# bxh1/VIDO-SLAM

Hardware: AMD Instinct MI355X
Metric: frames/sec end-to-end (flow+depth+track+local-BA) at 640x480; BA iters/sec (higher is better)
Workload: dtype f32

## Files before the change

### include/vido_c.h

```cpp
#ifndef VIDO_C_H
#define VIDO_C_H
#include <stdint.h>
#include <stddef.h>
#ifdef __cplusplus
extern "C" {
#endif

#define VIDO_OK              0
#define VIDO_E_INVALID      -1
#define VIDO_E_NO_DEVICE    -2
#define VIDO_E_HIP          -3
#define VIDO_E_CAPACITY     -4
#define VIDO_E_NOMEM        -5

#define VIDO_MAX_LEVELS 16

typedef struct vido_ctx vido_ctx;

typedef struct vido_keypoint { float x, y, size, angle, response; int32_t octave; } vido_keypoint;

typedef struct vido_config {
    int32_t device;
    int32_t width, height;
    int32_t max_batch;
// ... 126 lines not shown
    double* H_T;
    double* dyn_xyz;
    const int32_t* dyn_cam; const double* dyn_meas;
    const int32_t* tern_prev; const int32_t* tern_cur; const int32_t* tern_H;
    const int32_t* sm_i; const int32_t* sm_j;
    double info_dyn, info_tern, info_smooth, huber_dyn, huber_tern, huber_smooth;
} vido_ba_dynamic;
int vido_ba_optimize_dynamic(vido_ctx* ctx, vido_ba_problem* prob, vido_ba_dynamic* dyn, vido_ba_result* result,
                             vido_allreduce_fn allreduce, void* user);

int vido_correlation(vido_ctx* ctx, const float* first, const float* second, int B, int C, int H, int W, int stride,
                     float* out, int on_device);
int vido_det_order(vido_ctx* ctx, const float* scores, const long long* labels, const int* n_det, float confidence, int cap, long long* order, long long* labels_out, long long* n_live);
int vido_roi_levels(vido_ctx* ctx, const float* boxes, int n, float k_min, float k_max, int* out);
int vido_mask_logit_select(vido_ctx* ctx, const float* feat, const float* w, const float* b, const long long* labels, float* out, int n, int c, int hw, int classes);
int vido_bias_act(vido_ctx* ctx, float* x, const float* bias, int N, int C, int H, int W, float slope);
int vido_bias_unary(vido_ctx* ctx, float* x, const float* bias, int N, int C, int H, int W, int kind);
int vido_upcat_reflect(vido_ctx* ctx, const float* x, const float* skip, int C1, int C2, int h, int w, float* out);
int vido_minmax_norm_u16(vido_ctx* ctx, const float* d, const float* mm, int64_t n, int32_t* out);
int vido_bias_res_act(vido_ctx* ctx, float* x, const float* bias, const float* res, int N, int C, int H, int W, float slope);
int vido_area_feed(vido_ctx* ctx, const uint8_t* bgr, int H, int W, float* out, int OH, int OW, float div);
int vido_backwarp(vido_ctx* ctx, const float* x, const float* flow, int B, int C, int H, int W, float* out);
int vido_deconv4s2_depthwise(vido_ctx* ctx, const float* x, const float* weight, int B, int C, int H, int W, float input_slope, float* out);

int vido_conv1x1_supported(int cin, int cout, int hw);
int vido_conv1x1_layout(int cin, int cout, int hw);
int vido_conv1x1_set_arith(int arith);
int vido_conv1x1_range_flag(vido_ctx* ctx, int reset);
int vido_conv1x1_bias_act(vido_ctx* ctx, const float* x, const float* w_packed, const float* bias, const float* residual, float* y, int cin, int cout, int hw, float slope);
int vido_deconv2x2_supported(int n, int cin, int cout, int h, int w);
int vido_deconv2x2_bias_act(vido_ctx* ctx, const float* x, const float* w_packed, const float* bias, float* y, int n, int cin, int cout, int h, int w, float slope);
int vido_conv1x1_bias_up2_act(vido_ctx* ctx, const float* x, const float* w_packed, const float* bias, const float* residual_half, float* y, int cin, int cout, int h, int w, float slope);

int vido_conv_kxk_c2(vido_ctx* ctx, const float* x, const float* w, const float* bias, const float* residual, float* y, int cin, int k, int h, int w_);
int vido_conv1x1_skinny(vido_ctx* ctx, const float* x, const float* w_packed, const float* bias, const float* residual, float* y, int cin, int cout, long long hw, float slope);

int vido_conv_direct_supported(int cin, int cout, int h, int w, int kh, int kw, int sh, int sw, int ph, int pw);
long long vido_conv_direct_packed_floats(int cin, int cout, int kh, int kw);
int vido_conv_direct_pack(const float* w, int cin, int cout, int kh, int kw, float* w_packed);
int vido_conv_direct_bias_act(vido_ctx* ctx, const float* x, const float* w_packed, const float* bias, float* y, int n, int cin, int cout, int h, int w,
                              int kh, int kw, int sh, int sw, int ph, int pw, float slope);

int vido_wino3x3_supported(int cin, int cout, int h, int w);
int vido_wino3x3_fills_chip(int n, int cout, int h, int w, int min_wgs);
long long vido_wino3x3_packed_floats(int cin, int cout);
int vido_wino3x3_pack(const float* w, int cin, int cout, float* u_packed);
int vido_wino3x3_bias_act(vido_ctx* ctx, const float* x, const float* u_packed, const float* bias, float* y, int n, int cin, int cout, int h, int w, float slope);
int vido_wino3x3_form(int n, int cin, int cout, int h, int w);
int vido_fc_h_splitk(int rows, int k, int outs);
int vido_fc_h(vido_ctx* ctx, const float* x, const void* w_packed, const float* bias, float* part, float* y, int rows, int k, int outs, float slope);
int vido_conv3x3_h_supported(int n, int cin, int cout, int h, int w);
int vido_conv3x3_h_workgroups(int n, int cout, int h, int w);
int vido_conv3x3_h_bias_act(vido_ctx* ctx, const float* x, const void* w_packed, const float* bias, float* y, int n, int cin, int cout, int h, int w, float slope);
long long vido_wino3x3_packed_floats_form(int cin, int cout, int form);
int vido_wino3x3_pack_form(const float* w, int cin, int cout, int form, float* u_packed);
int vido_wino3x3_bias_act_form(vido_ctx* ctx, const float* x, const float* u_packed, const float* bias, float* y, int n, int cin, int cout, int h, int w, float slope, int form);
int vido_gconv3x3_supported(int H, int W, int cpg_in, int cpg_out);
int64_t vido_gconv3x3_packed_size(int groups, int cpg_in, int cpg_out);
int vido_gconv3x3_bias_act(vido_ctx* ctx, const float* x, const float* in_bias, const float* w_packed, const float* bias, float* y, int groups, int cpg_in, int cpg_out, int H, int W, float slope);
int vido_gconv3x3_s2_supported(int H, int W, int cpg_in, int cpg_out);
int vido_gconv3x3_s2_bias_act(vido_ctx* ctx, const float* x, const float* w_packed, const float* bias, float* y, int groups, int cpg_in, int cpg_out, int H, int W, float slope);
int vido_lfn_reg_front(vido_ctx* ctx, const float* im1, const float* im2, const float* flow, const float* mean, float scale, int B, int C, int H, int W, float* out, int out_channels);
int vido_lfn_reg_tail(vido_ctx* ctx, const float* dist, const float* flow, const float* wx, const float* bx, const float* wy, const float* by, int B, int K, int H, int W, float* out);
int vido_roi_align(vido_ctx* ctx, const float* feat, int B, int C, int H, int W, const float* rois, int n_rois,
                   float spatial_scale, int pooled_h, int pooled_w, int sampling_ratio, float* out, int on_device);
int vido_nms(vido_ctx* ctx, const float* boxes_xyxy, const float* scores, int n, float thresh, int32_t* keep_out,
             int32_t* n_keep, int on_device);
int vido_nms_grouped(vido_ctx* ctx, const float* boxes_xyxy, const float* scores, const int32_t* groups, int n, float thresh,
                     int32_t* keep_out, int32_t* n_keep, int on_device);
int vido_nms_segments(vido_ctx* ctx, const float* boxes_xyxy, const int32_t* groups, const int32_t* seg_off, const int32_t* seg_n, int n_seg, int max_n, int total,
                      float thresh, int32_t* keep_out, int32_t* n_keep);
int vido_roi_align_fpn(vido_ctx* ctx, const float* const feat[4], const int H[4], const int W[4], const float scale[4], int C, const float* boxes, const int32_t* level,
                       int n, int pooled_h, int pooled_w, int sampling_ratio, float* out);
int vido_nchw_to_nhwc(vido_ctx* ctx, const float* src, int B, int C, int H, int W, float* dst);
int vido_roi_align_fpn_nhwc(vido_ctx* ctx, const float* const feat[4], const int H[4], const int W[4], const float scale[4], int C, const float* boxes, const int32_t* level,
                            int n, int pooled_h, int pooled_w, int sampling_ratio, float* out);
int vido_bawin_create(vido_ctx* ctx, int cap_frames, int cap_features);
int vido_bawin_push_frame(vido_ctx* ctx, int frame, int n, const double* meas, const float* xyz, const int32_t* asso);
int vido_bawin_set_labels(vido_ctx* ctx, int n, const int32_t* quads);
int vido_bawin_solve(vido_ctx* ctx, int start, int N, vido_ba_problem* prob, vido_ba_result* res, int32_t* n_obs_out, int32_t* n_pt_out);
int vido_bawin_read_points(vido_ctx* ctx, int frame, int n, float* xyz_out);
int vido_rpn_select(vido_ctx* ctx, int n_levels, const float* const* logits, const float* const* deltas, const int* h, const int* w, const int* stride, const float* cell_anchors,
                    int A, int K, int img_w, int img_h, float* boxes_out, float* scores_out, int32_t* n_out);
int vido_rpn_merge(vido_ctx* ctx, const float* boxes, const float* scores, const int32_t* keep, const int32_t* cnt, int n_levels, int K, int post_nms_top_n, int n_final,
                   float* out_boxes, float* out_scores, int32_t* n_valid);
int vido_det_class_sort(vido_ctx* ctx, const float* prob, const float* deltas, const float* proposals, const float* objectness, int N, int nc, float thresh, const float weights[4],
                        int img_w, int img_h, float* seg_boxes, int32_t* order, int32_t* seg_n);
int vido_det_select(vido_ctx* ctx, const float* prob, const float* seg_boxes, const int32_t* order, const int32_t* keep, const int32_t* cnt, int N, int nc, int detections_per_img, int cap,
                    int32_t* scratch, float* out_boxes, float* out_scores, int64_t* out_labels, int32_t* n_det);
int vido_mask_label_image(vido_ctx* ctx, const float* masks, const float* boxes, const int64_t* labels, int n, int M, int padding, float thresh, int H, int W, uint8_t* out);
int vido_box_decode(vido_ctx* ctx, const float* deltas, const float* boxes, int n, int k, const float weights[4],
                    float* out, int on_device);

int vido_pnp_ransac(vido_ctx* ctx, const float* pts3d, const float* pts2d, int n, double fx, double fy, double cx, double cy,
                    int max_iters, double reproj_err, double confidence, uint64_t seed, double T_out[16], uint8_t* inlier_mask,
                    int32_t* n_inliers);

int vido_pnp_ransac_batch(vido_ctx* ctx, int n_prob, const float* const* pts3d, const float* const* pts2d, const int32_t* n, double fx, double fy, double cx, double cy,
                          int max_iters, double reproj_err, double confidence, const uint64_t* seeds, double* T_out, uint8_t* const* inlier_mask, int32_t* n_inliers);

typedef struct vido_host_maps { const int32_t* mask; const float* depth; const float* flow; int32_t width, height; } vido_host_maps;
float vido_depth_noise(float z, unsigned seed);
int vido_undistort_points(const float* xy, int n, const float K[4], const float dist[5], float* xy_out);
int vido_renew_static(const vido_host_maps* maps, const float* stat_xy, int n_stat, const int32_t* TM_sta, int n_tm, const float* sample_xy, int n_sample,
                      int max_num, int32_t* src_out, int32_t* inlier_out, float* flow_out, int cap, int32_t* n_out);
int vido_renew_objects(const vido_host_maps* maps, const float* obj_xy, const int32_t* obj_label, int n_obj_pts,
// ... 48 lines not shown
```

### vido-slam_amd/csrc/conv3x3h.hip

```cpp
#include "common.hpp"
#include <type_traits>

namespace {
typedef float f32x16 __attribute__((ext_vector_type(16)));
typedef float f32x2 __attribute__((ext_vector_type(2)));
typedef _Float16 f16x8 __attribute__((ext_vector_type(8)));
typedef _Float16 f16x2 __attribute__((ext_vector_type(2)));
typedef unsigned u32x4 __attribute__((ext_vector_type(4)));

#define C3_OOB 0x40000000u
#define C3_WSLOT 24576
#define C3_RBW 3
#define C3_WPIX(BR) (((BR) + 2) * 18)
#define C3_XP(BR) ((16 * C3_WPIX(BR) + 511) / 512)
#define C3_RAW(BR) (C3_XP(BR) * 8 * 256)
#define C3_PLANE(BR) (C3_WPIX(BR) * 32)
#define C3_PBUF(BR) (2 * C3_PLANE(BR))
#define C3_LDS(BR) (C3_RBW * C3_WSLOT + C3_RAW(BR) + 2 * C3_PBUF(BR))

struct C3Args { const float* x; const void* wp; const float* bias; float* y; int N, Cin, Cout, H, W, nby, nbx, mt, total, nchunk; float slope; unsigned wbytes; unsigned* range_flag; };

template <int RPW, int CG>
__global__ __launch_bounds__(512) void k_conv3x3_h(C3Args A)
{
    constexpr int BR = 16 / CG, MT = 32 * RPW * CG, WPIX = C3_WPIX(BR), XP = C3_XP(BR), RAWB = C3_RAW(BR), PLANE = C3_PLANE(BR), PBUF = C3_PBUF(BR), CK = (WPIX * 8 + 511) / 512, NMM = 9 * RPW, NRD = 2 * RPW + 2;
    extern __shared__ __attribute__((aligned(16))) char c3_lds[];
    char* L = c3_lds;
    const int tid = threadIdx.x, lane = tid & 63, w = __builtin_amdgcn_readfirstlane(tid >> 6);
    const int per = gridDim.x >> 3, item = (blockIdx.x & 7) * per + (blockIdx.x >> 3);
    if (item >= A.total) return;
    const int nt = item / A.mt, mtile = item - nt * A.mt, m0 = mtile * MT;
    const int bpi = A.nby * A.nbx, n = nt / bpi, brem = nt - n * bpi, by = brem / A.nbx, bx = brem - by * A.nbx, Y0 = by * BR, X0 = bx * 16;
    const int rp = CG == 1 ? w : (w & 3), rb0 = CG == 1 ? 0 : RPW * (w >> 2);
    const int hw = A.H * A.W, nsteps = A.nchunk * 3;

    const __amdgpu_buffer_rsrc_t wr = __builtin_amdgcn_make_buffer_rsrc((void*)A.wp, 0, A.wbytes, 0x00020000);
    const unsigned avo = 16u * (unsigned)lane;
    unsigned abase[3], avq[3];
#pragma unroll
    for (int q = 0; q < 3; q++) { const int i = w + 8 * q, rb = i / 6, rem = i - 6 * rb; abase[q] = 1024u * (unsigned)(((m0 >> 5) + rb) * A.nchunk * 18 + rem); avq[q] = rb < RPW * CG ? avo : 0x80000000u; }
    unsigned xvo[11];
#pragma unroll
    for (int j = 0; j < XP; j++) {
        const int e = 64 * (8 * j + w) + lane, ch = e / WPIX, rem = e - ch * WPIX, row = rem / 18, col = rem - row * 18, gy = Y0 - 1 + row, gx = X0 - 1 + col;
        xvo[j] = (e < 16 * WPIX && gy >= 0 && gy < A.H && gx >= 0 && gx < A.W) ? 4u * (unsigned)(ch * hw + gy * A.W + gx) : C3_OOB;
    }
    const unsigned ximg = 4u * (unsigned)n * (unsigned)A.Cin * (unsigned)hw, ximg_end = ximg + 4u * (unsigned)A.Cin * (unsigned)hw, xchunk = 64u * (unsigned)hw;
    char* const RAW = L + C3_RBW * C3_WSLOT;
    char* const PL = RAW + RAWB;
    auto issue_w = [&](int s, int slot) {
        char* S = L + slot * C3_WSLOT + w * 1024;
        const unsigned so = 6144u * (unsigned)s;
#pragma unroll
        for (int q = 0; q < 3; q++) __builtin_amdgcn_raw_ptr_buffer_load_lds(wr, (__attribute__((address_space(3))) void*)(S + q * 8192), 16, avq[q], abase[q] + so, 0, 0);
    };
    auto issue_x = [&](int c) {
        const unsigned so = ximg + xchunk * (unsigned)c;
        const __amdgpu_buffer_rsrc_t xc = __builtin_amdgcn_make_buffer_rsrc((void*)((const char*)A.x + so), 0, ximg_end - so, 0x00020000);
#pragma unroll
        for (int j = 0; j < XP; j++) __builtin_amdgcn_raw_ptr_buffer_load_lds(xc, (__attribute__((address_space(3))) void*)(RAW + (8 * j + w) * 256), 4, xvo[j], 0, 0, 0);
    };
    float xmax = 0.f;
    const f32x2 k2048 = {2048.f, 2048.f};
    auto convert = [&](int buf) {
        const float* R = (const float*)RAW;
        unsigned* P = (unsigned*)(PL + buf * PBUF);
#pragma unroll
        for (int k = 0; k < CK; k++) {
            const int idx = tid + 512 * k;
            if (k < CK - 1 || idx < WPIX * 8) {
                const int q = idx / WPIX, pix = idx - q * WPIX;
                const f32x2 v = {R[(2 * q) * WPIX + pix], R[(2 * q + 1) * WPIX + pix]};
                const f16x2 h = __builtin_convertvector(v, f16x2);
                f32x2 vs, r;
                asm("v_pk_mul_f32 %0, %1, %2" : "=v"(vs) : "v"(v), "v"(k2048));
                asm("v_fma_mix_f32 %0, %1, %2, %3 op_sel_hi:[1,0,0]" : "=v"(r.x) : "v"(h), "s"(-2048.f), "v"(vs.x));
                asm("v_fma_mix_f32 %0, %1, %2, %3 op_sel:[1,0,0] op_sel_hi:[1,0,0]" : "=v"(r.y) : "v"(h), "s"(-2048.f), "v"(vs.y));
                const f16x2 l = __builtin_convertvector(r, f16x2);
                P[pix * 8 + q] = __builtin_bit_cast(unsigned, h); P[PLANE / 4 + pix * 8 + q] = __builtin_bit_cast(unsigned, l);
                xmax = __builtin_elementwise_maximum(__builtin_elementwise_maximum(xmax, __builtin_fabsf(v.x)), __builtin_fabsf(v.y));
            }
        }
    };

    f32x16 acc[RPW], acl[RPW];
#pragma unroll
    for (int rb = 0; rb < RPW; rb++)
#pragma unroll
        for (int r = 0; r < 16; r++) { acc[rb][r] = 0.f; acl[rb][r] = 0.f; }
    typedef const __attribute__((address_space(3))) char* lds_c;
    const unsigned a_lane = 16u * (unsigned)lane;
    const unsigned b_lane = (unsigned)(C3_RBW * C3_WSLOT + RAWB) + 32u * (unsigned)((2 * rp + ((lane & 31) >> 4)) * 18 + (lane & 15)) + 16u * (unsigned)(lane >> 5);

    issue_x(0); issue_w(0, 0); issue_w(min(1, nsteps - 1), 1);
    asm volatile("s_waitcnt vmcnt(6) lgkmcnt(0)\n\ts_barrier" ::: "memory");
    convert(0);
    int slot = 0;
    u32x4 a[2][RPW][2], b[2][2];
    auto step = [&](auto dy_c, auto nbuf_c, int pbuf, auto&& copies) {
        constexpr int dy = decltype(dy_c)::value, NBUF = decltype(nbuf_c)::value;
        lds_c Ab = (lds_c)(L + slot * C3_WSLOT) + a_lane;
        lds_c Bb = (lds_c)L + b_lane + pbuf * PBUF + dy * (18 * 32);
        auto ld = [&](int dx, int set) {
#pragma unroll
            for (int rb = 0; rb < RPW; rb++)
#pragma unroll
                for (int pl = 0; pl < 2; pl++) a[set][rb][pl] = *(const __attribute__((address_space(3))) u32x4*)(Ab + (((rb0 + rb) * 3 + dx) * 2 + pl) * 1024);
#pragma unroll
            for (int pl = 0; pl < 2; pl++) b[set][pl] = *(const __attribute__((address_space(3))) u32x4*)(Bb + dx * 32 + pl * PLANE);
        };
        __builtin_amdgcn_sched_barrier(0);
        ld(0, 0);
        copies();
#pragma unroll
        for (int dx = 0; dx < 3; dx++) {
            if (dx < 2) ld(dx + 1, (dx + 1) & 1);
#pragma unroll
            for (int term = 0; term < 3; term++) {
                constexpr int PA[3] = {0, 1, 0}, PB[3] = {1, 0, 0};
#pragma unroll
                for (int rb = 0; rb < RPW; rb++) {
                    f32x16& d = term == 2 ? acc[rb] : acl[rb];
                    d = __builtin_amdgcn_mfma_f32_32x32x16_f16(__builtin_bit_cast(f16x8, a[dx & 1][rb][PA[term]]), __builtin_bit_cast(f16x8, b[dx & 1][PB[term]]), d, 0, 0, 0);
                }
            }
        }
        __builtin_amdgcn_sched_group_barrier(0x100, NRD, 0);
#pragma unroll
        for (int i = 0; i < NMM; i++) {
            __builtin_amdgcn_sched_group_barrier(0x008, 1, 0);
            if (i < 2 * NRD) __builtin_amdgcn_sched_group_barrier(0x100, 1, 0);
            if (i >= 1 && i < 1 + NBUF) __builtin_amdgcn_sched_group_barrier(0x020, 1, 0);
        }
        __builtin_amdgcn_sched_barrier(0);
    };
    for (int c = 0; c < A.nchunk; c++) {
        const int pbuf = c & 1, cn = min(c + 1, A.nchunk - 1);
        asm volatile("s_waitcnt vmcnt(3) lgkmcnt(0)\n\ts_barrier" ::: "memory");
        step(std::integral_constant<int, 0>{}, std::integral_constant<int, 3 + XP>{}, pbuf, [&] { const int sf = slot == 0 ? C3_RBW - 1 : slot - 1; issue_w(min(3 * c + 2, nsteps - 1), sf); issue_x(cn); });
        slot = slot + 1 == C3_RBW ? 0 : slot + 1;
        asm volatile("s_waitcnt vmcnt(%0) lgkmcnt(0)\n\ts_barrier" :: "n"(3 + XP) : "memory");
        step(std::integral_constant<int, 1>{}, std::integral_constant<int, 3>{}, pbuf, [&] { const int sf = slot == 0 ? C3_RBW - 1 : slot - 1; issue_w(min(3 * c + 3, nsteps - 1), sf); });
        slot = slot + 1 == C3_RBW ? 0 : slot + 1;
        asm volatile("s_waitcnt vmcnt(3) lgkmcnt(0)\n\ts_barrier" ::: "memory");
        step(std::integral_constant<int, 2>{}, std::integral_constant<int, 3>{}, pbuf, [&] { const int sf = slot == 0 ? C3_RBW - 1 : slot - 1; issue_w(min(3 * c + 4, nsteps - 1), sf); });
        convert(pbuf ^ 1);
        slot = slot + 1 == C3_RBW ? 0 : slot + 1;
    }
    asm volatile("s_waitcnt vmcnt(0) lgkmcnt(0)" ::: "memory");
#pragma unroll
    for (int rb = 0; rb < RPW; rb++) acc[rb] += acl[rb] * 0x1p-11f;
    if (!(xmax < 65504.f) && A.range_flag) atomicOr(A.range_flag, 1u);

    const float* wsc = (const float*)((const char*)A.wp + (size_t)A.nchunk * 16 * 18 * A.Cout * 2);
    const int p = lane & 31, Y = Y0 + 2 * rp + (p >> 4), X = X0 + (p & 15);
    const bool inside = Y < A.H && X < A.W;
    float* yb = A.y + (size_t)n * A.Cout * hw + (size_t)Y * A.W + X;
#pragma unroll
    for (int rb = 0; rb < RPW; rb++) {
        float bv[16], sv[16];
#pragma unroll
        for (int r = 0; r < 16; r++) { const int co = m0 + 32 * (rb0 + rb) + 8 * (r >> 2) + 4 * (lane >> 5) + (r & 3); bv[r] = A.bias ? A.bias[co] : 0.f; sv[r] = wsc[co]; }
        if (inside) {
#pragma unroll
            for (int r = 0; r < 16; r++) {
                const int co = m0 + 32 * (rb0 + rb) + 8 * (r >> 2) + 4 * (lane >> 5) + (r & 3);
                const float v = acc[rb][r] * sv[r] + bv[r];
                yb[(size_t)co * hw] = fmaxf(v, v * A.slope);
            }
        }
    }
}
}

extern "C" {

int vido_conv3x3_h_supported(int n, int cin, int cout, int h, int w)
{
    const long long cp = (cin + 15) / 16 * 16;
    return n >= 1 && cin >= 1 && (cout == 32 || cout == 64 || (cout >= 128 && cout % 128 == 0)) && h >= 1 && w >= 1 && 4ll * n * cin * h * w < (1ll << 30) && 4ll * n * cout * h * w < (1ll << 30)
           && 36ll * cp * cout < (1ll << 31);
}

#define C3_MIN16 190
static int c3_block_rows(int n, int cout, int h, int w)
{
    static const int force = [] { const char* e = getenv("VIDO_CONV3X3_H_ROWS"); return e ? atoi(e) : 0; }();
    if (cout == 32) return 16;
    if (force == 16 || force == 8) return force;
    const int mt = cout >= 128 ? cout / 128 : 1;
    return n * ((h + 15) / 16) * ((w + 15) / 16) * mt >= C3_MIN16 ? 16 : 8;
}
int vido_conv3x3_h_workgroups(int n, int cout, int h, int w) { const int br = c3_block_rows(n, cout, h, w); return n * ((h + br - 1) / br) * ((w + 15) / 16) * (cout >= 128 ? cout / 128 : 1); }

int vido_conv3x3_h_bias_act(vido_ctx* ctx, const float* x, const void* w_packed, const float* bias, float* y, int n, int cin, int cout, int h, int w, float slope)
{
    if (!ctx) return VIDO_E_INVALID;
    if (!x || !w_packed || !y || x == y || !vido_conv3x3_h_supported(n, cin, cout, h, w) || slope < 0.f || slope > 1.f || (((uintptr_t)x | (uintptr_t)y) & 3) || ((uintptr_t)w_packed & 15))
        return vido_set_error(ctx, VIDO_E_INVALID, "conv3x3_h: no kernel for %d x %d -> %d channels at %d x %d (or a pointer is misaligned, or slope outside [0, 1])", n, cin, cout, h, w);
    HIP_TRY(ctx, hipSetDevice(ctx->device));
    hipStream_t st = ctx->has_ext_stream ? ctx->ext_stream : ctx->stream;
    const int br = c3_block_rows(n, cout, h, w);
    const int nby = (h + br - 1) / br, nbx = (w + 15) / 16, mt = cout >= 128 ? cout / 128 : 1, total = n * nby * nbx * mt;
    const int nchunk = (cin + 15) / 16;
    C3Args A{x, w_packed, bias, y, n, cin, cout, h, w, nby, nbx, mt, total, nchunk, slope, (unsigned)(36ll * 16 * nchunk * cout), ctx->c1_range_flag};
    static bool attr[64] = {};
    if (!attr[ctx->device & 63]) {
#define C3_ATTR(RPW_, CG_) HIP_TRY(ctx, hipFuncSetAttribute((const void*)k_conv3x3_h<RPW_, CG_>, hipFuncAttributeMaxDynamicSharedMemorySize, (int)C3_LDS(16 / CG_)))
        C3_ATTR(4, 1); C3_ATTR(2, 2); C3_ATTR(2, 1); C3_ATTR(1, 2); C3_ATTR(1, 1);
#undef C3_ATTR
        attr[ctx->device & 63] = true;
    }
    const dim3 grid(8 * ((total + 7) / 8));
#define C3_LAUNCH(RPW_, CG_) hipLaunchKernelGGL((k_conv3x3_h<RPW_, CG_>), grid, dim3(512), C3_LDS(16 / CG_), st, A)
    if (cout >= 128) { if (br == 16) C3_LAUNCH(4, 1); else C3_LAUNCH(2, 2); }
    else if (cout == 64) { if (br == 16) C3_LAUNCH(2, 1); else C3_LAUNCH(1, 2); }
    else C3_LAUNCH(1, 1);
#undef C3_LAUNCH
    HIP_TRY(ctx, hipGetLastError());
    return VIDO_OK;
}

}
```

### vido-slam_amd/nets/ops.py

```python
import ctypes as C
import os
import torch

_WINO_MIN_WGS = int(os.environ.get("VIDO_WINO_MIN_WGS", "0"))
_CONV3X3_H_MIN_WGS = 0 if os.environ.get("VIDO_CONV3X3_H") == "0" else int(os.environ.get("VIDO_CONV3X3_H_MIN_WGS", "128"))
_CONVDIRECT_SET = os.environ.get("VIDO_CONVDIRECT_SET", "novalu")


def correlation_torch_reference(first, second, stride):
    a, b = first[:, :, ::stride, ::stride], second[:, :, ::stride, ::stride]
    pad = torch.nn.functional.pad(b, (3, 3, 3, 3))
    H, W = a.shape[2], a.shape[3]
    return torch.stack([(a * pad[:, :, p:p + H, o:o + W]).mean(1) for p in range(7) for o in range(7)], 1)


class HipOps:

    def __init__(self, ctx):
        self.ctx = ctx

    def _adopt_stream(self):
        st = torch.cuda.current_stream().cuda_stream
        self.ctx._check(self.ctx.lib.vido_set_stream(self.ctx.h, C.c_void_p(st), 1))

    def correlation(self, first, second, stride):
        if not first.is_cuda:
            raise RuntimeError("HipOps.correlation needs CUDA(HIP) tensors; there is no CPU fallback")
        first = first.contiguous().float(); second = second.contiguous().float()
        B, Cc, H, W = first.shape
        out = torch.empty((B, 49, (H + stride - 1) // stride, (W + stride - 1) // stride), device=first.device, dtype=torch.float32)
        self._adopt_stream()
        self.ctx._check(self.ctx.lib.vido_correlation(self.ctx.h, C.c_void_p(first.data_ptr()), C.c_void_p(second.data_ptr()), B, Cc, H, W, stride,
                                                      C.c_void_p(out.data_ptr()), 1))
        return out

    def bias_act_(self, x, bias, slope):
        assert x.is_cuda and x.is_contiguous() and x.dtype == torch.float32
        N, Cc, H, W = x.shape
        self._adopt_stream()
        self.ctx._check(self.ctx.lib.vido_bias_act(self.ctx.h, C.c_void_p(x.data_ptr()), C.c_void_p(bias.data_ptr()), N, Cc, H, W, C.c_float(slope)))
        return x

    def deconv2x2_conv(self, conv, x, slope):
        w = conv.weight
        if (tuple(w.shape[2:]) != (2, 2) or tuple(conv.stride) != (2, 2) or tuple(conv.padding) != (0, 0) or tuple(conv.output_padding) != (0, 0) or tuple(conv.dilation) != (1, 1)
                or conv.groups != 1 or not x.is_cuda or x.dtype != torch.float32 or os.environ.get("VIDO_NO_DECONV_H")):
            return None
        n, cin, H, W = (int(v) for v in x.shape); cout = int(w.shape[1])
        if not self.ctx.lib.vido_deconv2x2_supported(n, cin, cout, H, W):
            return None
        key = (w.data_ptr(), w._version, str(x.device))
        if getattr(conv, "_dc_key", None) != key:
            conv._dc_w = pack_deconv2x2(w).to(x.device); conv._dc_key = key
        out = torch.empty((n, cout, 2 * H, 2 * W), device=x.device, dtype=torch.float32)
        self.gconv_flops = getattr(self, "gconv_flops", 0.0) + 2.0 * n * cin * cout * 4 * H * W
        self._adopt_stream()
        b = conv.bias
        self.ctx._check(self.ctx.lib.vido_deconv2x2_bias_act(self.ctx.h, C.c_void_p(x.contiguous().data_ptr()), C.c_void_p(conv._dc_w.data_ptr()), C.c_void_p(b.data_ptr()) if b is not None else None,
                                                             C.c_void_p(out.data_ptr()), n, cin, cout, H, W, C.c_float(slope)))
# ... 183 lines not shown
        self._adopt_stream()
        self.ctx._check(self.ctx.lib.vido_conv_kxk_c2(self.ctx.h, C.c_void_p(x.data_ptr()), C.c_void_p(wc.data_ptr()), C.c_void_p(conv.bias.data_ptr()) if conv.bias is not None else None,
                                                      C.c_void_p(residual.data_ptr()) if residual is not None else None, C.c_void_p(out.data_ptr()), int(cin), k, int(H), int(W)))
        return out

    def conv1x1_skinny(self, x, w_packed, bias, cout, slope=1.0, residual=None):
        assert x.is_cuda and x.dtype == torch.float32 and x.shape[0] == 1
        x = x.contiguous(); cin, H, W = int(x.shape[1]), int(x.shape[2]), int(x.shape[3])
        out = torch.empty((1, cout, H, W), device=x.device, dtype=torch.float32)
        if residual is not None:
            residual = residual.contiguous(); assert residual.shape == out.shape
        self.gconv_flops = getattr(self, "gconv_flops", 0.0) + 2.0 * cout * cin * H * W
        self._adopt_stream()
        self.ctx._check(self.ctx.lib.vido_conv1x1_skinny(self.ctx.h, C.c_void_p(x.data_ptr()), C.c_void_p(w_packed.data_ptr()), C.c_void_p(bias.data_ptr()) if bias is not None else None,
                                                         C.c_void_p(residual.data_ptr()) if residual is not None else None, C.c_void_p(out.data_ptr()), cin, int(cout), C.c_longlong(H * W), C.c_float(slope)))
        return out

    def conv1x1_skinny_conv(self, conv, x, slope=1.0):
        w = conv.weight
        cout, cin = int(w.shape[0]), int(w.shape[1])
        if (tuple(w.shape[2:]) != (1, 1) or tuple(conv.stride) != (1, 1) or tuple(conv.padding) != (0, 0) or conv.groups != 1 or cin % 2 or cin > 256 or cout > 256
                or not x.is_cuda or x.shape[0] != 1 or x.dtype != torch.float32):
            return None
        key = (w.data_ptr(), w._version, str(x.device))
        if getattr(conv, "_c1s_key", None) != key:
            conv._c1s_w = pack_conv1x1_skinny(w).to(x.device); conv._c1s_key = key
        return self.conv1x1_skinny(x, conv._c1s_w, conv.bias, cout, slope)

    def wino3x3_supported(self, cin, cout, H, W):
        return bool(self.ctx.lib.vido_wino3x3_supported(int(cin), int(cout), int(H), int(W)))

    def wino3x3_form(self, N, cin, cout, H, W):
        return int(self.ctx.lib.vido_wino3x3_form(int(N), int(cin), int(cout), int(H), int(W)))

    def wino3x3_bias_act(self, x, u_packed, bias, cout, slope=1.0, form=0):
        assert x.is_cuda and x.is_contiguous() and x.dtype == torch.float32 and u_packed.is_cuda
        N, cin, H, W = x.shape
        out = torch.empty((N, cout, H, W), device=x.device, dtype=torch.float32)
        self.gconv_flops = getattr(self, "gconv_flops", 0.0) + 2.0 * N * cout * cin * 9 * H * W
        self._adopt_stream()
        self.ctx._check(self.ctx.lib.vido_wino3x3_bias_act_form(self.ctx.h, C.c_void_p(x.data_ptr()), C.c_void_p(u_packed.data_ptr()), C.c_void_p(bias.data_ptr()) if bias is not None else None,
                                                                C.c_void_p(out.data_ptr()), int(N), int(cin), int(cout), int(H), int(W), C.c_float(slope), int(form)))
        return out

    def wino3x3_conv(self, conv, x, slope, weight=None, bias=None):
        w = conv.weight if weight is None else weight
        b = conv.bias if bias is None and weight is None else bias
        if (tuple(w.shape[2:]) != (3, 3) or tuple(conv.stride) != (1, 1) or tuple(conv.padding) != (1, 1) or tuple(conv.dilation) != (1, 1) or conv.groups != 1
                or getattr(conv, "padding_mode", "zeros") != "zeros" or not x.is_cuda or not self.wino3x3_supported(w.shape[1], w.shape[0], x.shape[2], x.shape[3])
                or 4 * x.numel() >= 1 << 30 or 4 * x.shape[0] * w.shape[0] * x.shape[2] * x.shape[3] >= 1 << 30):
            return None
        if _WINO_MIN_WGS > 0 and not self.ctx.lib.vido_wino3x3_fills_chip(int(x.shape[0]), int(w.shape[0]), int(x.shape[2]), int(x.shape[3]), _WINO_MIN_WGS):
            return None
        if (_CONV3X3_H_MIN_WGS > 0 and x.dtype == torch.float32 and self.ctx.lib.vido_conv3x3_h_supported(int(x.shape[0]), int(w.shape[1]), int(w.shape[0]), int(x.shape[2]), int(x.shape[3]))
                and self.ctx.lib.vido_conv3x3_h_workgroups(int(x.shape[0]), int(w.shape[0]), int(x.shape[2]), int(x.shape[3])) >= (1 if int(w.shape[0]) == 64 else _CONV3X3_H_MIN_WGS)):
            key = (w.data_ptr(), w._version, str(x.device))
            if getattr(conv, "_c3h_key", None) != key:
                conv._c3h_w = pack_conv3x3_h(w).to(x.device); conv._c3h_key = key
            return self.conv3x3_h_bias_act(x.contiguous(), conv._c3h_w, b, int(w.shape[0]), slope)
        form = self.wino3x3_form(x.shape[0], w.shape[1], w.shape[0], x.shape[2], x.shape[3])
        key = (w.data_ptr(), w._version, str(x.device))
        if getattr(conv, "_wino_key", None) != key:
            conv._wino_u = {}; conv._wino_key = key
        if form not in conv._wino_u:
            conv._wino_u[form] = pack_wino3x3(w, form).to(x.device)
        return self.wino3x3_bias_act(x.contiguous(), conv._wino_u[form], b, int(w.shape[0]), slope, form)

    def conv3x3_h_bias_act(self, x, w_packed, bias, cout, slope):
        assert x.is_cuda and x.is_contiguous() and x.dtype == torch.float32
        N, cin, H, W = x.shape
        assert w_packed.dtype == torch.int16 and w_packed.numel() == 2 * cout * ((cin + 15) // 16 * 16 * 9 + 1), "conv3x3_h: weight not packed by pack_conv3x3_h for this layer"
        out = torch.empty((N, cout, H, W), device=x.device, dtype=torch.float32)
        self.gconv_flops = getattr(self, "gconv_flops", 0.0) + 2.0 * N * cout * cin * 9 * H * W
        self._adopt_stream()
        self.ctx._check(self.ctx.lib.vido_conv3x3_h_bias_act(self.ctx.h, C.c_void_p(x.data_ptr()), C.c_void_p(w_packed.data_ptr()), C.c_void_p(bias.data_ptr()) if bias is not None else None,
                                                             C.c_void_p(out.data_ptr()), int(N), int(cin), int(cout), int(H), int(W), C.c_float(slope)))
        return out

    def fc_h(self, x, w_packed, bias, outs, slope=1.0):
        assert x.is_cuda and x.is_contiguous() and x.dtype == torch.float32 and x.dim() == 2
        rows, k = int(x.shape[0]), int(x.shape[1])
        S = int(self.ctx.lib.vido_fc_h_splitk(rows, k, int(outs)))
        if S <= 0:
            return None
        assert w_packed.dtype == torch.int16 and w_packed.numel() == 2 * outs * (k + 1), "fc_h: weight not packed (pack_conv1x1(w[:, :, None, None], 3))"
        part = torch.empty((S, rows, outs), device=x.device, dtype=torch.float32); y = torch.empty((rows, outs), device=x.device, dtype=torch.float32)
        self.gconv_flops = getattr(self, "gconv_flops", 0.0) + 2.0 * rows * k * outs
        self._adopt_stream()
        self.ctx._check(self.ctx.lib.vido_fc_h(self.ctx.h, C.c_void_p(x.data_ptr()), C.c_void_p(w_packed.data_ptr()), C.c_void_p(bias.data_ptr()) if bias is not None else None,
                                               C.c_void_p(part.data_ptr()), C.c_void_p(y.data_ptr()), rows, k, int(outs), C.c_float(slope)))
        return y

    def fc_h_linear(self, lin, x, slope=1.0):
        w = lin.weight
        if not x.is_cuda or x.dtype != torch.float32 or x.dim() != 2 or os.environ.get("VIDO_NO_FC_H") or int(self.ctx.lib.vido_fc_h_splitk(int(x.shape[0]), int(w.shape[1]), int(w.shape[0]))) <= 0:
            return None
        key = (w.data_ptr(), w._version, str(x.device))
        if getattr(lin, "_fch_key", None) != key:
            lin._fch_w = pack_conv1x1(w.detach().reshape(int(w.shape[0]), int(w.shape[1]), 1, 1), 3).to(x.device); lin._fch_key = key
        return self.fc_h(x.contiguous(), lin._fch_w, lin.bias, int(w.shape[0]), slope)

    def conv_direct_conv(self, conv, x, slope):
        w = conv.weight
        kh, kw = int(w.shape[2]), int(w.shape[3]); sh, sw = (int(v) for v in conv.stride); ph, pw = (int(v) for v in conv.padding)
        if _CONVDIRECT_SET == "novalu" and (kh, kw) in ((3, 3), (7, 7)) and int(w.shape[0]) >= 32:
            return None
        if (tuple(conv.dilation) != (1, 1) or conv.groups != 1 or getattr(conv, "padding_mode", "zeros") != "zeros" or not x.is_cuda or x.dtype != torch.float32
                or not self.ctx.lib.vido_conv_direct_supported(int(w.shape[1]), int(w.shape[0]), int(x.shape[2]), int(x.shape[3]), kh, kw, sh, sw, ph, pw)
                or 4 * x.numel() >= 1 << 30):
            return None
        N, cin, H, W = x.shape; cout = int(w.shape[0])
        Ho, Wo = (H + 2 * ph - kh) // sh + 1, (W + 2 * pw - kw) // sw + 1
        if 4 * N * cout * Ho * Wo >= 1 << 30:
            return None
        key = (w.data_ptr(), w._version, str(x.device))
        if getattr(conv, "_cd_key", None) != key:
            conv._cd_w = pack_conv_direct(w).to(x.device); conv._cd_key = key
        x = x.contiguous()
        out = torch.empty((N, cout, Ho, Wo), device=x.device, dtype=torch.float32)
        self.gconv_flops = getattr(self, "gconv_flops", 0.0) + 2.0 * N * cout * cin * kh * kw * Ho * Wo
        self._adopt_stream()
        b = conv.bias
        self.ctx._check(self.ctx.lib.vido_conv_direct_bias_act(self.ctx.h, C.c_void_p(x.data_ptr()), C.c_void_p(conv._cd_w.data_ptr()), C.c_void_p(b.data_ptr()) if b is not None else None,
                                                               C.c_void_p(out.data_ptr()), int(N), int(cin), cout, int(H), int(W), kh, kw, sh, sw, ph, pw, C.c_float(slope)))
        return out

    def lfn_reg_front(self, im1, im2, flow, scale, feat):
# ... 314 lines not shown
```

Measured before the change: 126.0.

## Add split-K mode to conv3x3_h for small-tile layers with reduce kernel

Adds a K-split path to the half-precision 3x3 convolution kernel. When a layer has fewer than 128 output tiles, the input-channel chunks are divided across several workgroups. Each workgroup writes scaled partial sums to a scratch buffer, and a vectorized reduce kernel then sums them and applies bias and leaky-ReLU. The aim is to fill the chip on small, deep layers, which previously fell back to Winograd or underused the CUs. The cost is extra partial-buffer memory traffic, an additional kernel launch and an allocation per call.

```diff
diff --git a/include/vido_c.h b/include/vido_c.h
--- a/include/vido_c.h
+++ b/include/vido_c.h
@@ -202,6 +202,8 @@
 int vido_conv3x3_h_supported(int n, int cin, int cout, int h, int w);
 int vido_conv3x3_h_workgroups(int n, int cout, int h, int w);
 int vido_conv3x3_h_bias_act(vido_ctx* ctx, const float* x, const void* w_packed, const float* bias, float* y, int n, int cin, int cout, int h, int w, float slope);
+int vido_conv3x3_h_ksplit(int n, int cin, int cout, int h, int w);
+int vido_conv3x3_h_bias_act_ksplit(vido_ctx* ctx, const float* x, const void* w_packed, const float* bias, float* part, float* y, int n, int cin, int cout, int h, int w, float slope, int splits);
 long long vido_wino3x3_packed_floats_form(int cin, int cout, int form);
 int vido_wino3x3_pack_form(const float* w, int cin, int cout, int form, float* u_packed);
 int vido_wino3x3_bias_act_form(vido_ctx* ctx, const float* x, const float* u_packed, const float* bias, float* y, int n, int cin, int cout, int h, int w, float slope, int form);
diff --git a/vido-slam_amd/csrc/conv3x3h.hip b/vido-slam_amd/csrc/conv3x3h.hip
--- a/vido-slam_amd/csrc/conv3x3h.hip
+++ b/vido-slam_amd/csrc/conv3x3h.hip
@@ -18,9 +18,9 @@
 #define C3_PBUF(BR) (2 * C3_PLANE(BR))
 #define C3_LDS(BR) (C3_RBW * C3_WSLOT + C3_RAW(BR) + 2 * C3_PBUF(BR))
 
-struct C3Args { const float* x; const void* wp; const float* bias; float* y; int N, Cin, Cout, H, W, nby, nbx, mt, total, nchunk; float slope; unsigned wbytes; unsigned* range_flag; };
-
-template <int RPW, int CG>
+struct C3Args { const float* x; const void* wp; const float* bias; float* y; int N, Cin, Cout, H, W, nby, nbx, mt, total, nchunk, tiles, cps; float slope; unsigned wbytes; unsigned* range_flag; };
+
+template <int RPW, int CG, bool PART>
 __global__ __launch_bounds__(512) void k_conv3x3_h(C3Args A)
 {
     constexpr int BR = 16 / CG, MT = 32 * RPW * CG, WPIX = C3_WPIX(BR), XP = C3_XP(BR), RAWB = C3_RAW(BR), PLANE = C3_PLANE(BR), PBUF = C3_PBUF(BR), CK = (WPIX * 8 + 511) / 512, NMM = 9 * RPW, NRD = 2 * RPW + 2;
@@ -29,10 +29,11 @@
     const int tid = threadIdx.x, lane = tid & 63, w = __builtin_amdgcn_readfirstlane(tid >> 6);
     const int per = gridDim.x >> 3, item = (blockIdx.x & 7) * per + (blockIdx.x >> 3);
     if (item >= A.total) return;
-    const int nt = item / A.mt, mtile = item - nt * A.mt, m0 = mtile * MT;
+    const int ks = item / A.tiles, ti = item - ks * A.tiles, cb = ks * A.cps, ce = min(cb + A.cps, A.nchunk);
+    const int nt = ti / A.mt, mtile = ti - nt * A.mt, m0 = mtile * MT;
     const int bpi = A.nby * A.nbx, n = nt / bpi, brem = nt - n * bpi, by = brem / A.nbx, bx = brem - by * A.nbx, Y0 = by * BR, X0 = bx * 16;
     const int rp = CG == 1 ? w : (w & 3), rb0 = CG == 1 ? 0 : RPW * (w >> 2);
-    const int hw = A.H * A.W, nsteps = A.nchunk * 3;
+    const int hw = A.H * A.W, slast = 3 * ce - 1;
 
     const __amdgpu_buffer_rsrc_t wr = __builtin_amdgcn_make_buffer_rsrc((void*)A.wp, 0, A.wbytes, 0x00020000);
     const unsigned avo = 16u * (unsigned)lane;
@@ -92,7 +93,7 @@
     const unsigned a_lane = 16u * (unsigned)lane;
     const unsigned b_lane = (unsigned)(C3_RBW * C3_WSLOT + RAWB) + 32u * (unsigned)((2 * rp + ((lane & 31) >> 4)) * 18 + (lane & 15)) + 16u * (unsigned)(lane >> 5);
 
-    issue_x(0); issue_w(0, 0); issue_w(min(1, nsteps - 1), 1);
+    issue_x(cb); issue_w(3 * cb, 0); issue_w(min(3 * cb + 1, slast), 1);
     asm volatile("s_waitcnt vmcnt(6) lgkmcnt(0)\n\ts_barrier" ::: "memory");
     convert(0);
     int slot = 0;
@@ -134,16 +135,16 @@
         }
         __builtin_amdgcn_sched_barrier(0);
     };
-    for (int c = 0; c < A.nchunk; c++) {
-        const int pbuf = c & 1, cn = min(c + 1, A.nchunk - 1);
+    for (int c = cb; c < ce; c++) {
+        const int pbuf = (c - cb) & 1, cn = min(c + 1, ce - 1);
         asm volatile("s_waitcnt vmcnt(3) lgkmcnt(0)\n\ts_barrier" ::: "memory");
-        step(std::integral_constant<int, 0>{}, std::integral_constant<int, 3 + XP>{}, pbuf, [&] { const int sf = slot == 0 ? C3_RBW - 1 : slot - 1; issue_w(min(3 * c + 2, nsteps - 1), sf); issue_x(cn); });
+        step(std::integral_constant<int, 0>{}, std::integral_constant<int, 3 + XP>{}, pbuf, [&] { const int sf = slot == 0 ? C3_RBW - 1 : slot - 1; issue_w(min(3 * c + 2, slast), sf); issue_x(cn); });
         slot = slot + 1 == C3_RBW ? 0 : slot + 1;
         asm volatile("s_waitcnt vmcnt(%0) lgkmcnt(0)\n\ts_barrier" :: "n"(3 + XP) : "memory");
-        step(std::integral_constant<int, 1>{}, std::integral_constant<int, 3>{}, pbuf, [&] { const int sf = slot == 0 ? C3_RBW - 1 : slot - 1; issue_w(min(3 * c + 3, nsteps - 1), sf); });
+        step(std::integral_constant<int, 1>{}, std::integral_constant<int, 3>{}, pbuf, [&] { const int sf = slot == 0 ? C3_RBW - 1 : slot - 1; issue_w(min(3 * c + 3, slast), sf); });
         slot = slot + 1 == C3_RBW ? 0 : slot + 1;
         asm volatile("s_waitcnt vmcnt(3) lgkmcnt(0)\n\ts_barrier" ::: "memory");
-        step(std::integral_constant<int, 2>{}, std::integral_constant<int, 3>{}, pbuf, [&] { const int sf = slot == 0 ? C3_RBW - 1 : slot - 1; issue_w(min(3 * c + 4, nsteps - 1), sf); });
+        step(std::integral_constant<int, 2>{}, std::integral_constant<int, 3>{}, pbuf, [&] { const int sf = slot == 0 ? C3_RBW - 1 : slot - 1; issue_w(min(3 * c + 4, slast), sf); });
         convert(pbuf ^ 1);
         slot = slot + 1 == C3_RBW ? 0 : slot + 1;
     }
@@ -155,21 +156,43 @@
     const float* wsc = (const float*)((const char*)A.wp + (size_t)A.nchunk * 16 * 18 * A.Cout * 2);
     const int p = lane & 31, Y = Y0 + 2 * rp + (p >> 4), X = X0 + (p & 15);
     const bool inside = Y < A.H && X < A.W;
-    float* yb = A.y + (size_t)n * A.Cout * hw + (size_t)Y * A.W + X;
+    float* yb = A.y + ((size_t)(PART ? ks * A.N : 0) + n) * A.Cout * hw + (size_t)Y * A.W + X;
 #pragma unroll
     for (int rb = 0; rb < RPW; rb++) {
         float bv[16], sv[16];
 #pragma unroll
-        for (int r = 0; r < 16; r++) { const int co = m0 + 32 * (rb0 + rb) + 8 * (r >> 2) + 4 * (lane >> 5) + (r & 3); bv[r] = A.bias ? A.bias[co] : 0.f; sv[r] = wsc[co]; }
+        for (int r = 0; r < 16; r++) { const int co = m0 + 32 * (rb0 + rb) + 8 * (r >> 2) + 4 * (lane >> 5) + (r & 3); bv[r] = !PART && A.bias ? A.bias[co] : 0.f; sv[r] = wsc[co]; }
         if (inside) {
 #pragma unroll
             for (int r = 0; r < 16; r++) {
                 const int co = m0 + 32 * (rb0 + rb) + 8 * (r >> 2) + 4 * (lane >> 5) + (r & 3);
+                if (PART) { yb[(size_t)co * hw] = acc[rb][r] * sv[r]; continue; }
                 const float v = acc[rb][r] * sv[r] + bv[r];
                 yb[(size_t)co * hw] = fmaxf(v, v * A.slope);
             }
         }
     }
+}
+
+template <int V>
+__global__ __launch_bounds__(256) void k_conv3x3_h_reduce(const float* __restrict__ part, const float* __restrict__ bias, float* __restrict__ y, long long nv, int hwv, int cout, int S, float slope)
+{
+    typedef float fv __attribute__((ext_vector_type(V)));
+    const long long i = (long long)blockIdx.x * 256 + threadIdx.x;
+    if (i >= nv) return;
+    const fv* P = (const fv*)part;
+    fv v = P[i];
+    int s = 1;
+    for (; s + 8 <= S; s += 8) {
+        fv t[8];
+#pragma unroll
+        for (int j = 0; j < 8; j++) t[j] = P[i + (long long)(s + j) * nv];
+#pragma unroll
+        for (int j = 0; j < 8; j++) v += t[j];
+    }
+    for (; s < S; s++) v += P[i + (long long)s * nv];
+    if (bias) v += bias[(int)((i / hwv) % cout)];
+    ((fv*)y)[i] = __builtin_elementwise_max(v, v * slope);
 }
 }
 
@@ -193,32 +216,69 @@
 }
 int vido_conv3x3_h_workgroups(int n, int cout, int h, int w) { const int br = c3_block_rows(n, cout, h, w); return n * ((h + br - 1) / br) * ((w + 15) / 16) * (cout >= 128 ? cout / 128 : 1); }
 
-int vido_conv3x3_h_bias_act(vido_ctx* ctx, const float* x, const void* w_packed, const float* bias, float* y, int n, int cin, int cout, int h, int w, float slope)
+#define C3_KSPLIT_BELOW 128
+#define C3_CUS 256
+int vido_conv3x3_h_ksplit(int n, int cin, int cout, int h, int w)
+{
+    if (!vido_conv3x3_h_supported(n, cin, cout, h, w)) return 0;
+    const int tiles = vido_conv3x3_h_workgroups(n, cout, h, w), nchunk = (cin + 15) / 16;
+    if (tiles >= C3_KSPLIT_BELOW) return 1;
+    int S = min(nchunk, max(1, C3_CUS / tiles));
+    const int cps = (nchunk + S - 1) / S;
+    S = (nchunk + cps - 1) / cps;
+    while (S > 1 && 4ll * S * n * cout * h * w >= (1ll << 31)) S--;
+    return S >= 3 ? S : 1;
+}
+
+static int c3_launch(vido_ctx* ctx, const float* x, const void* w_packed, const float* bias, float* part, float* y, int n, int cin, int cout, int h, int w, float slope, int S)
 {
     if (!ctx) return VIDO_E_INVALID;
+    const int nchunk = (cin + 15) / 16;
     if (!x || !w_packed || !y || x == y || !vido_conv3x3_h_supported(n, cin, cout, h, w) || slope < 0.f || slope > 1.f || (((uintptr_t)x | (uintptr_t)y) & 3) || ((uintptr_t)w_packed & 15))
         return vido_set_error(ctx, VIDO_E_INVALID, "conv3x3_h: no kernel for %d x %d -> %d channels at %d x %d (or a pointer is misaligned, or slope outside [0, 1])", n, cin, cout, h, w);
+    if (S < 1 || S > nchunk || (S > 1 && (!part || part == x || part == y || ((uintptr_t)part & 15) || ((uintptr_t)y & 15) || 4ll * S * n * cout * h * w >= (1ll << 31))))
+        return vido_set_error(ctx, VIDO_E_INVALID, "conv3x3_h: %d K slices for %d input chunks (or the partial-sum buffer is missing, misaligned or too large)", S, nchunk);
     HIP_TRY(ctx, hipSetDevice(ctx->device));
     hipStream_t st = ctx->has_ext_stream ? ctx->ext_stream : ctx->stream;
     const int br = c3_block_rows(n, cout, h, w);
-    const int nby = (h + br - 1) / br, nbx = (w + 15) / 16, mt = cout >= 128 ? cout / 128 : 1, total = n * nby * nbx * mt;
-    const int nchunk = (cin + 15) / 16;
-    C3Args A{x, w_packed, bias, y, n, cin, cout, h, w, nby, nbx, mt, total, nchunk, slope, (unsigned)(36ll * 16 * nchunk * cout), ctx->c1_range_flag};
+    const int nby = (h + br - 1) / br, nbx = (w + 15) / 16, mt = cout >= 128 ? cout / 128 : 1, tiles = n * nby * nbx * mt;
+    const int cps = (nchunk + S - 1) / S;
+    S = (nchunk + cps - 1) / cps;
+    C3Args A{x, w_packed, bias, S > 1 ? part : y, n, cin, cout, h, w, nby, nbx, mt, tiles * S, nchunk, tiles, cps, slope, (unsigned)(36ll * 16 * nchunk * cout), ctx->c1_range_flag};
     static bool attr[64] = {};
     if (!attr[ctx->device & 63]) {
-#define C3_ATTR(RPW_, CG_) HIP_TRY(ctx, hipFuncSetAttribute((const void*)k_conv3x3_h<RPW_, CG_>, hipFuncAttributeMaxDynamicSharedMemorySize, (int)C3_LDS(16 / CG_)))
+#define C3_ATTR(RPW_, CG_) HIP_TRY(ctx, hipFuncSetAttribute((const void*)k_conv3x3_h<RPW_, CG_, false>, hipFuncAttributeMaxDynamicSharedMemorySize, (int)C3_LDS(16 / CG_))); \
+                           HIP_TRY(ctx, hipFuncSetAttribute((const void*)k_conv3x3_h<RPW_, CG_, true>, hipFuncAttributeMaxDynamicSharedMemorySize, (int)C3_LDS(16 / CG_)))
         C3_ATTR(4, 1); C3_ATTR(2, 2); C3_ATTR(2, 1); C3_ATTR(1, 2); C3_ATTR(1, 1);
 #undef C3_ATTR
         attr[ctx->device & 63] = true;
     }
-    const dim3 grid(8 * ((total + 7) / 8));
-#define C3_LAUNCH(RPW_, CG_) hipLaunchKernelGGL((k_conv3x3_h<RPW_, CG_>), grid, dim3(512), C3_LDS(16 / CG_), st, A)
+    const dim3 grid(8 * ((A.total + 7) / 8));
+#define C3_LAUNCH(RPW_, CG_) do { if (S > 1) hipLaunchKernelGGL((k_conv3x3_h<RPW_, CG_, true>), grid, dim3(512), C3_LDS(16 / CG_), st, A); \
+                                  else hipLaunchKernelGGL((k_conv3x3_h<RPW_, CG_, false>), grid, dim3(512), C3_LDS(16 / CG_), st, A); } while (0)
     if (cout >= 128) { if (br == 16) C3_LAUNCH(4, 1); else C3_LAUNCH(2, 2); }
     else if (cout == 64) { if (br == 16) C3_LAUNCH(2, 1); else C3_LAUNCH(1, 2); }
     else C3_LAUNCH(1, 1);
 #undef C3_LAUNCH
     HIP_TRY(ctx, hipGetLastError());
+    if (S > 1) {
+        const int hw = h * w;
+        const long long e = (long long)n * cout * hw;
+        if (hw % 4 == 0) hipLaunchKernelGGL(k_conv3x3_h_reduce<4>, dim3((unsigned)((e / 4 + 255) / 256)), dim3(256), 0, st, (const float*)part, bias, y, e / 4, hw / 4, cout, S, slope);
+        else hipLaunchKernelGGL(k_conv3x3_h_reduce<1>, dim3((unsigned)((e + 255) / 256)), dim3(256), 0, st, (const float*)part, bias, y, e, hw, cout, S, slope);
+        HIP_TRY(ctx, hipGetLastError());
+    }
     return VIDO_OK;
 }
 
-}
+int vido_conv3x3_h_bias_act(vido_ctx* ctx, const float* x, const void* w_packed, const float* bias, float* y, int n, int cin, int cout, int h, int w, float slope)
+{
+    return c3_launch(ctx, x, w_packed, bias, nullptr, y, n, cin, cout, h, w, slope, 1);
+}
+
+int vido_conv3x3_h_bias_act_ksplit(vido_ctx* ctx, const float* x, const void* w_packed, const float* bias, float* part, float* y, int n, int cin, int cout, int h, int w, float slope, int splits)
+{
+    return c3_launch(ctx, x, w_packed, bias, part, y, n, cin, cout, h, w, slope, splits);
+}
+
+}
diff --git a/vido-slam_amd/nets/ops.py b/vido-slam_amd/nets/ops.py
--- a/vido-slam_amd/nets/ops.py
+++ b/vido-slam_amd/nets/ops.py
@@ -5,6 +5,7 @@
 _WINO_MIN_WGS = int(os.environ.get("VIDO_WINO_MIN_WGS", "0"))
 _CONV3X3_H_MIN_WGS = 0 if os.environ.get("VIDO_CONV3X3_H") == "0" else int(os.environ.get("VIDO_CONV3X3_H_MIN_WGS", "128"))
 _CONVDIRECT_SET = os.environ.get("VIDO_CONVDIRECT_SET", "novalu")
+_CONV3X3_H_KSPLIT = os.environ.get("VIDO_CONV3X3_H_KSPLIT", "1") != "0"
 
 
 def correlation_torch_reference(first, second, stride):
@@ -294,12 +295,14 @@
             return None
         if _WINO_MIN_WGS > 0 and not self.ctx.lib.vido_wino3x3_fills_chip(int(x.shape[0]), int(w.shape[0]), int(x.shape[2]), int(x.shape[3]), _WINO_MIN_WGS):
             return None
-        if (_CONV3X3_H_MIN_WGS > 0 and x.dtype == torch.float32 and self.ctx.lib.vido_conv3x3_h_supported(int(x.shape[0]), int(w.shape[1]), int(w.shape[0]), int(x.shape[2]), int(x.shape[3]))
-                and self.ctx.lib.vido_conv3x3_h_workgroups(int(x.shape[0]), int(w.shape[0]), int(x.shape[2]), int(x.shape[3])) >= (1 if int(w.shape[0]) == 64 else _CONV3X3_H_MIN_WGS)):
-            key = (w.data_ptr(), w._version, str(x.device))
-            if getattr(conv, "_c3h_key", None) != key:
-                conv._c3h_w = pack_conv3x3_h(w).to(x.device); conv._c3h_key = key
-            return self.conv3x3_h_bias_act(x.contiguous(), conv._c3h_w, b, int(w.shape[0]), slope)
+        shape = (int(x.shape[0]), int(w.shape[1]), int(w.shape[0]), int(x.shape[2]), int(x.shape[3]))
+        if _CONV3X3_H_MIN_WGS > 0 and x.dtype == torch.float32 and self.ctx.lib.vido_conv3x3_h_supported(*shape):
+            splits = int(self.ctx.lib.vido_conv3x3_h_ksplit(*shape)) if _CONV3X3_H_KSPLIT and _WINO_MIN_WGS == 0 else 1
+            if splits > 1 or self.ctx.lib.vido_conv3x3_h_workgroups(shape[0], shape[2], shape[3], shape[4]) >= (1 if shape[2] == 64 else _CONV3X3_H_MIN_WGS):
+                key = (w.data_ptr(), w._version, str(x.device))
+                if getattr(conv, "_c3h_key", None) != key:
+                    conv._c3h_w = pack_conv3x3_h(w).to(x.device); conv._c3h_key = key
+                return self.conv3x3_h_bias_act(x.contiguous(), conv._c3h_w, b, shape[2], slope, splits)
         form = self.wino3x3_form(x.shape[0], w.shape[1], w.shape[0], x.shape[2], x.shape[3])
         key = (w.data_ptr(), w._version, str(x.device))
         if getattr(conv, "_wino_key", None) != key:
@@ -308,13 +311,19 @@
             conv._wino_u[form] = pack_wino3x3(w, form).to(x.device)
         return self.wino3x3_bias_act(x.contiguous(), conv._wino_u[form], b, int(w.shape[0]), slope, form)
 
-    def conv3x3_h_bias_act(self, x, w_packed, bias, cout, slope):
+    def conv3x3_h_bias_act(self, x, w_packed, bias, cout, slope, splits=1):
         assert x.is_cuda and x.is_contiguous() and x.dtype == torch.float32
         N, cin, H, W = x.shape
         assert w_packed.dtype == torch.int16 and w_packed.numel() == 2 * cout * ((cin + 15) // 16 * 16 * 9 + 1), "conv3x3_h: weight not packed by pack_conv3x3_h for this layer"
         out = torch.empty((N, cout, H, W), device=x.device, dtype=torch.float32)
         self.gconv_flops = getattr(self, "gconv_flops", 0.0) + 2.0 * N * cout * cin * 9 * H * W
         self._adopt_stream()
+        if splits > 1:
+            part = torch.empty((int(splits), N, cout, H, W), device=x.device, dtype=torch.float32)
+            self.ctx._check(self.ctx.lib.vido_conv3x3_h_bias_act_ksplit(self.ctx.h, C.c_void_p(x.data_ptr()), C.c_void_p(w_packed.data_ptr()),
+                                                                        C.c_void_p(bias.data_ptr()) if bias is not None else None, C.c_void_p(part.data_ptr()),
+                                                                        C.c_void_p(out.data_ptr()), int(N), int(cin), int(cout), int(H), int(W), C.c_float(slope), int(splits)))
+            return out
         self.ctx._check(self.ctx.lib.vido_conv3x3_h_bias_act(self.ctx.h, C.c_void_p(x.data_ptr()), C.c_void_p(w_packed.data_ptr()), C.c_void_p(bias.data_ptr()) if bias is not None else None,
                                                              C.c_void_p(out.data_ptr()), int(N), int(cin), int(cout), int(H), int(W), C.c_float(slope)))
         return out
```

New measurement: 127.7, median of 6. 1.01x the previous value.
